# RenYurui/Global-Flow-Local-Attention

Measured on NVIDIA H100. Metric: warp-layer Mpixels/s (fwd+bwd) @256^2 C=256 k=5, higher is better.
Workload: dtype bf16

## Files before the change

global-flow-local-attention_b200/csrc/local_attn_bwd_tc.cu:

```cuda
#include <mutex>

#include "det_accum.cuh"
#include "tile_window.cuh"

namespace gfla {
namespace tc {

constexpr int BT_THREADS = 256;
constexpr int BT_PIX_REGS = 168, BT_GS_REGS = 88;
constexpr int BT_BAR_PASS = 1;
constexpr int BT_BAR_PIX = 2;
constexpr int BT_BAR_GS = 3;
constexpr int BT_BAR_FULL = 4;
constexpr int BT_BAR_FREE = 7;
constexpr int BT_AWSTR = 128 * 2 + 16;
constexpr int BT_PSTR = SEG + 1;

constexpr int BT_NAW = 3;

template <int CN>
struct BwdSmem {
    static constexpr int GSTR = CN * 2 + 16;
    static constexpr int G = 0;
    static constexpr int S = G + 128 * GSTR;
    static constexpr int AW = S + 2 * SEG * GSTR;
    static constexpr int P = AW + BT_NAW * SEG * BT_AWSTR;
    static constexpr int IRR = P + 128 * BT_PSTR * 4;
    static constexpr int ROWS = IRR + 129 * 4;
    static constexpr int ALLOC = ROWS + BT_NAW * 4;
};

__device__ __forceinline__ void red_add_16x8(__nv_bfloat16* p, const uint32_t (&v)[4]) {
    asm volatile("red.global.add.noftz.v4.bf16x2 [%0], {%1, %2, %3, %4};" ::"l"(p), "r"(v[0]), "r"(v[1]), "r"(v[2]), "r"(v[3])
                 : "memory");
}
__device__ __forceinline__ void red_add_16x8(__half* p, const uint32_t (&v)[4]) {
    asm volatile("red.global.add.noftz.v4.f16x2 [%0], {%1, %2, %3, %4};" ::"l"(p), "r"(v[0]), "r"(v[1]), "r"(v[2]), "r"(v[3])
                 : "memory");
}

__device__ __forceinline__ void quad_transpose(uint32_t (&v)[4], int t) {
    const bool t1 = (t & 2) != 0, t0 = (t & 1) != 0;
    uint32_t y0 = __shfl_xor_sync(0xffffffffu, t1 ? v[0] : v[2], 2);
    uint32_t y1 = __shfl_xor_sync(0xffffffffu, t1 ? v[1] : v[3], 2);
    if (t1) { v[0] = y0; v[1] = y1; } else { v[2] = y0; v[3] = y1; }
    y0 = __shfl_xor_sync(0xffffffffu, t0 ? v[0] : v[1], 1);
    y1 = __shfl_xor_sync(0xffffffffu, t0 ? v[2] : v[3], 1);
    if (t0) { v[0] = y0; v[2] = y1; } else { v[1] = y0; v[3] = y1; }
}

template <typename T, int CN, bool M0, bool M1>
__device__ __forceinline__ void p_gemm(uint32_t ga, uint32_t sf, float (&pacc)[2][2][4]) {
    constexpr int GSTR = BwdSmem<CN>::GSTR;
#pragma unroll 4
    for (int kk = 0; kk < CN / 16; ++kk) {
        uint32_t a0[4], a1[4], bf[4];
        if (M0) ldsm_x4(ga + kk * 32, a0);
        if (M1) ldsm_x4(ga + 16 * GSTR + kk * 32, a1);
        ldsm_x4(sf + kk * 32, bf);
        if (M0) {
            mma16<T>(pacc[0][0], a0, bf[0], bf[1]);
            mma16<T>(pacc[0][1], a0, bf[2], bf[3]);
        }
        if (M1) {
            mma16<T>(pacc[1][0], a1, bf[0], bf[1]);
            mma16<T>(pacc[1][1], a1, bf[2], bf[3]);
        }
    }
}

__device__ __forceinline__ int border_slot(int y, int x, int Hs, int Ws) {
    if (y == 0) return x;
    if (y == Hs - 1) return Ws + x;
    if (x == 0) return 2 * Ws + y;
    if (x == Ws - 1) return 2 * Ws + Hs + y;
    return -1;
}

template <typename T, int CN>
__device__ __forceinline__ void load_g_tile(uint32_t g_base, const T* __restrict__ go_b, int c0, int C, int gx0, int gy0,
                                            int H, int W, int tid) {
    constexpr int GSTR = BwdSmem<CN>::GSTR;
#pragma unroll 4
    for (int i = 0; i < CN / 16; ++i) {
        const int idx = i * BT_THREADS + tid, m = idx / (CN / 8), j = idx % (CN / 8);
        const int qx = gx0 + (m & 15), qy = gy0 + (m >> 4);
        const bool in = qx < W && qy < H;
        cp_async16(g_base + m * GSTR + j * 16, in ? go_b + ((long long)qy * W + qx) * C + c0 + j * 8 : go_b, in ? 16u : 0u);
    }
    cp_async_commit();
}

template <typename T, int K, bool DET>
__device__ __forceinline__ void irregular_pixel_bwd(const T* __restrict__ src, const float* __restrict__ flow, const T* __restrict__ logits,
                                                    const T* __restrict__ gout, T* __restrict__ gsrc, float* __restrict__ gflow,
                                                    T* __restrict__ glogits, int b, int C, int Hs, int Ws, int H, int W,
                                                    int qx, int qy, int accumulate, int lane, fx_t* __restrict__ gsum,
                                                    double2 fsc) {
    constexpr int KK = K * K;
    const long long hw = (long long)H * W, qofs = (long long)qy * W + qx;
    const float fx = flow[(long long)b * 2 * hw + qofs], fy = flow[(long long)b * 2 * hw + hw + qofs];
    float p[KK], dp[KK];
    pixel_softmax<T, float, KK>(logits + (long long)b * KK * hw + qofs, hw, KK, p);
    const float inv_kk = 1.0f / static_cast<float>(KK);
    const T* s = src + (long long)b * Hs * Ws * C;
    using GS = std::conditional_t<DET, fx_t, T>;
    GS* gs;
    if constexpr (DET) gs = gsum + (long long)b * Hs * Ws * C;
    else gs = gsrc + (long long)b * Hs * Ws * C;
    const T* go = gout + ((long long)b * hw + qofs) * C;
    float gfx = 0.f, gfy = 0.f;
#pragma unroll
    for (int i = 0; i < K; ++i) {
        const AxisTap<float> ty = axis_tap<float>(fy, i - K / 2, qy, Hs);
#pragma unroll
        for (int j = 0; j < K; ++j) {
            const AxisTap<float> tx = axis_tap<float>(fx, j - K / 2, qx, Ws);
            const long long oLT = ((long long)ty.lo * Ws + tx.lo) * C, oRT = ((long long)ty.lo * Ws + tx.hi) * C,
                            oLB = ((long long)ty.hi * Ws + tx.lo) * C, oRB = ((long long)ty.hi * Ws + tx.hi) * C;
            const float pij = p[i * K + j] * inv_kk;
            float q[4] = {0.f, 0.f, 0.f, 0.f};
            for (int c = lane; c < C; c += 32) {
                const float g = ld(go + c);
                q[0] += g * ld(s + oLT + c);
                q[1] += g * ld(s + oRT + c);
                q[2] += g * ld(s + oLB + c);
                q[3] += g * ld(s + oRB + c);
                const float gp = g * pij;
                scatter_add<DET>(gs + oLT + c, gp * (tx.wlo * ty.wlo), fsc);
                scatter_add<DET>(gs + oRT + c, gp * (tx.whi * ty.wlo), fsc);
                scatter_add<DET>(gs + oLB + c, gp * (tx.wlo * ty.whi), fsc);
                scatter_add<DET>(gs + oRB + c, gp * (tx.whi * ty.whi), fsc);
            }
#pragma unroll
            for (int t = 0; t < 4; ++t)
#pragma unroll
                for (int o = 16; o > 0; o >>= 1) q[t] += __shfl_xor_sync(0xffffffffu, q[t], o);
            dp[i * K + j] = tap_backward<float>(tx, ty, pij, inv_kk, q[0], q[1], q[2], q[3], gfx, gfy);
        }
    }
    if (lane == 0)
        store_pixel_grads<T, float, float, KK>(p, dp, KK, gfx, gfy, glogits + (long long)b * KK * hw + qofs,
                                               gflow + (long long)b * 2 * hw + qofs, hw, accumulate);
}

template <int K, int CN, bool DET, typename T>
__global__ void __launch_bounds__(BT_THREADS, 2)
k_local_attn_bwd_tc(const T* __restrict__ src, const float* __restrict__ flow, const T* __restrict__ logits, const T* __restrict__ gout,
                    T* __restrict__ gsrc, float* __restrict__ gflow, T* __restrict__ glogits, float* __restrict__ gborder, int C, int Hs, int Ws, int H, int W, int gcols,
                    int grows, int accumulate, fx_t* __restrict__ gsum, const int* __restrict__ fx_exp) {
    constexpr int K1 = K + 1, KK = K * K;
    using L = BwdSmem<CN>;
    constexpr int GSTR = L::GSTR, NTW = CN / 32;
    extern __shared__ __align__(16) unsigned char smem[];
    int* irr = reinterpret_cast<int*>(smem + L::IRR);
    int& nirr = irr[128];
    unsigned char* rows = smem + L::ROWS;
    const int tid = threadIdx.x, lane = tid & 31, warp = tid >> 5, gid = lane >> 2, tig = lane & 3;
    const float inv_kk = 1.0f / static_cast<float>(KK);
    const uint32_t sb = smem_u32(smem);
    const uint32_t g_base = sb + L::G, s_base = sb + L::S, aw_base = sb + L::AW, p_base = sb + L::P;

    for (int i = tid; i < BT_NAW * SEG * 16; i += BT_THREADS) sts128(aw_base + (i >> 4) * BT_AWSTR + (i & 15) * 16, 0u, 0u, 0u, 0u);
    if (tid == 0) nirr = 0;
    __syncthreads();
    if (warp < 4) {
        setmaxnreg_inc<BT_PIX_REGS>();
        uint32_t b;
        int gx0, gy0, bx0, by0, bx1, by1;
        group_decode(gcols, grows, b, gx0, gy0);
        group_bbox<K>(flow, b, gx0, gy0, H, W, Hs, Ws, lane, bx0, by0, bx1, by1);
        const long long hw = (long long)H * W;
        const T* go_b = gout + (long long)b * hw * C;
        const int px = gx0 + (tid & 15), py = gy0 + (tid >> 4);
        const bool valid = px < W && py < H;
        const long long pofs = (long long)py * W + px;
        uint32_t w[K1 * K1 / 2];
        float Q[K1 * K1];
#pragma unroll
        for (int i = 0; i < K1 * K1; ++i) Q[i] = 0.f;
        int X0 = 0, Y0 = 0, X0u = 0, Y0u = 0;
        bool regular = false;
        if (valid) {
            float p[KK];
            pixel_softmax<T, float, KK>(logits + (long long)b * KK * hw + pofs, hw, KK, p);
            AxisTap<float> tx[K], ty[K];
            regular = taps_regular<float, K>(flow[(long long)b * 2 * hw + pofs], flow[(long long)b * 2 * hw + hw + pofs], px, py, Hs, Ws, tx, ty);
            if (regular) {
                X0u = tx[0].fl;
                Y0u = ty[0].fl;
                build_window<T, K>(p, tx, ty, Hs, Ws, inv_kk, w, X0, Y0);
            } else {
                irr[atomicAdd(&nirr, 1)] = tid;
            }
        }
        const T* s_b = src + (long long)b * Hs * Ws * C;
        const uint32_t g_frag_a = g_base + (warp * 32 + (lane & 15)) * GSTR + (lane >> 4) * 16;
        const uint32_t s_frag_b = s_base + ((lane & 7) + ((lane >> 4) << 3)) * GSTR + ((lane >> 3) & 1) * 16;

        for (int c0 = 0; c0 < C; c0 += CN) {
            if (c0 != 0) bar_sync(BT_BAR_PASS, BT_THREADS);
            load_g_tile<T, CN>(g_base, go_b, c0, C, gx0, gy0, H, W, tid);
            {
                const int i = tid >> 3;
                for (int j = tid & 7; j < CN / 8; j += 8)
                    cp_async16(s_base + i * GSTR + j * 16, s_b + ((long long)by0 * Ws + min(bx0 + i, Ws - 1)) * C + c0 + j * 8);
            }
            cp_async_commit();
            cp_async_wait<1>();
            bar_sync(BT_BAR_PASS, BT_THREADS);
            int s = 0;
            for (int a = 0, y = by0, x = bx0; y <= by1; ++s) {
                const int buf = s & 1;
                const int an = a == BT_NAW - 1 ? 0 : a + 1;
                int xn = x + SEG, yn = y;
                if (xn > bx1) { xn = bx0; ++yn; }
                if (s >= BT_NAW) bar_sync(BT_BAR_FREE + a, BT_THREADS);
                const bool act = regular && window_meets_step<K>(X0u, Y0u, Hs, Ws, y, x);
                if (act) scatter_window_row<K>(aw_base + a * (SEG * BT_AWSTR) + tid * 2, BT_AWSTR, w, X0, Y0, y, x);
                const uint32_t pm = warp_row_bits(act);
                if (lane == 0) rows[a * 4 + warp] = static_cast<unsigned char>(pm);
                bar_arrive(BT_BAR_FULL + a, BT_THREADS);
                cp_async_wait_all();
                bar_sync(BT_BAR_PIX, 128);
                if (yn <= by1) {
                    const int i = tid >> 3;
                    const uint32_t dst = s_base + (buf ^ 1) * (SEG * GSTR) + i * GSTR;
                    const T* sp = s_b + ((long long)yn * Ws + min(xn + i, Ws - 1)) * C + c0;
                    for (int j = tid & 7; j < CN / 8; j += 8) cp_async16(dst + j * 16, sp + j * 8);
                    cp_async_commit();
                }
                if (pm != 0u) {
                    float pacc[2][2][4];
#pragma unroll
                    for (int mt = 0; mt < 2; ++mt)
#pragma unroll
                        for (int nt = 0; nt < 2; ++nt)
#pragma unroll
                            for (int q = 0; q < 4; ++q) pacc[mt][nt][q] = 0.f;
                    const uint32_t sf = s_frag_b + buf * (SEG * GSTR);
                    if (pm == 3u) p_gemm<T, CN, true, true>(g_frag_a, sf, pacc);
                    else if (pm == 1u) p_gemm<T, CN, true, false>(g_frag_a, sf, pacc);
                    else p_gemm<T, CN, false, true>(g_frag_a, sf, pacc);
#pragma unroll
                    for (int mt = 0; mt < 2; ++mt) {
                        if (((pm >> mt) & 1u) == 0u) continue;
#pragma unroll
                        for (int h = 0; h < 2; ++h) {
                            const uint32_t row = p_base + (warp * 32 + mt * 16 + gid + 8 * h) * (BT_PSTR * 4);
#pragma unroll
                            for (int nt = 0; nt < 2; ++nt) {
                                stsf(row + (nt * 8 + 2 * tig) * 4, pacc[mt][nt][2 * h]);
                                stsf(row + (nt * 8 + 2 * tig + 1) * 4, pacc[mt][nt][2 * h + 1]);
                            }
                        }
                    }
                    __syncwarp();
                    if (act) {
                        const uint32_t prow = p_base + tid * (BT_PSTR * 4);
#pragma unroll
                        for (int r = 0; r < K1; ++r) {
                            if (clampi(Y0u + r, Hs - 1) != y) continue;
#pragma unroll
                            for (int t = 0; t < K1; ++t) {
                                const int e = clampi(X0u + t, Ws - 1) - x;
                                if (e >= 0 && e < SEG) Q[r * K1 + t] += ldsf(prow + e * 4);
                            }
                        }
                    }
                }
                x = xn;
                y = yn;
                a = an;
            }
            for (int j = max(s - BT_NAW, 0); j < s; ++j) bar_sync(BT_BAR_FREE + j % BT_NAW, BT_THREADS);
        }

        if (regular) {
            float p[KK], dp[KK];
            pixel_softmax<T, float, KK>(logits + (long long)b * KK * hw + pofs, hw, KK, p);
            AxisTap<float> tx[K], ty[K];
            taps_regular<float, K>(flow[(long long)b * 2 * hw + pofs], flow[(long long)b * 2 * hw + hw + pofs], px, py, Hs, Ws, tx, ty);
            float gfx = 0.f, gfy = 0.f;
#pragma unroll
            for (int i = 0; i < K; ++i)
#pragma unroll
                for (int j = 0; j < K; ++j)
                    dp[i * K + j] = tap_backward<float>(tx[j], ty[i], p[i * K + j] * inv_kk, inv_kk, Q[i * K1 + j], Q[i * K1 + j + 1],
                                                        Q[(i + 1) * K1 + j], Q[(i + 1) * K1 + j + 1], gfx, gfy);
            store_pixel_grads<T, float, float, KK>(p, dp, KK, gfx, gfy, glogits + (long long)b * KK * hw + pofs,
                                                   gflow + (long long)b * 2 * hw + pofs, hw, accumulate);
        }
        const double2 fsc = DET ? fx_scale(fx_exp[b]) : make_double2(0.0, 0.0);
        for (int i = warp; i < nirr; i += 4) {
            const int m = irr[i];
            irregular_pixel_bwd<T, K, DET>(src, flow, logits, gout, gsrc, gflow, glogits, b, C, Hs, Ws, H, W, gx0 + (m & 15),
                                        gy0 + (m >> 4), accumulate, lane, gsum, fsc);
        }
    } else {
        setmaxnreg_dec<BT_GS_REGS>();
        uint32_t b;
        int gx0, gy0, bx0, by0, bx1, by1;
        group_decode(gcols, grows, b, gx0, gy0);
        group_bbox<K>(flow, b, gx0, gy0, H, W, Hs, Ws, lane, bx0, by0, bx1, by1);
        const long long hw = (long long)H * W;
        const T* go_b = gout + (long long)b * hw * C;
        const int v = warp - 4, t = tid - 128;
        const uint32_t aw_frag = aw_base + (lane & 15) * BT_AWSTR + (lane >> 4) * 16;
        const uint32_t g_frag_b = g_base + (lane & 15) * GSTR + (v * (CN / 4) + (lane >> 4) * 8) * 2;
        T* gs_b = gsrc + (long long)b * Hs * Ws * C;
        fx_t* gx_b = nullptr;
        double2 fsc = make_double2(0.0, 0.0);
        if constexpr (DET) {
            gx_b = gsum + (long long)b * Hs * Ws * C;
            fsc = fx_scale(fx_exp[b]);
        }

        for (int c0 = 0; c0 < C; c0 += CN) {
            if (c0 != 0) bar_sync(BT_BAR_PASS, BT_THREADS);
            load_g_tile<T, CN>(g_base, go_b, c0, C, gx0, gy0, H, W, tid);
            cp_async_wait_all();
            bar_sync(BT_BAR_PASS, BT_THREADS);
            for (int a = 0, y = by0, x = bx0; y <= by1;) {
                const int an = a == BT_NAW - 1 ? 0 : a + 1;
                int xn = x + SEG, yn = y;
                if (xn > bx1) { xn = bx0; ++yn; }
                bar_sync(BT_BAR_FULL + a, BT_THREADS);
                const uint32_t grows_on = *reinterpret_cast<const uint32_t*>(rows + a * 4);
                if (grows_on == 0u) {
                    bar_arrive(BT_BAR_FREE + a, BT_THREADS);
                } else {
                    float gacc[NTW][4];
#pragma unroll
                    for (int nt = 0; nt < NTW; ++nt)
#pragma unroll
                        for (int q = 0; q < 4; ++q) gacc[nt][q] = 0.f;
#pragma unroll
                    for (int kk = 0; kk < 128 / 16; ++kk) {
                        if (((grows_on >> (8 * (kk >> 1) + (kk & 1))) & 1u) == 0u) continue;
                        uint32_t af[4];
                        ldsm_x4(aw_frag + a * (SEG * BT_AWSTR) + kk * 32, af);
#pragma unroll
                        for (int np = 0; np < NTW / 2; ++np) {
                            uint32_t bg[4];
                            ldsm_x4_t(g_frag_b + kk * 16 * GSTR + np * 32, bg);
                            mma16<T>(gacc[2 * np], af, bg[0], bg[1]);
                            mma16<T>(gacc[2 * np + 1], af, bg[2], bg[3]);
                        }
                    }
                    bar_sync(BT_BAR_GS, 128);
                    {
                        const uint32_t z = aw_base + a * (SEG * BT_AWSTR) + (t >> 3) * BT_AWSTR + (t & 7) * 32;
                        sts128(z, 0u, 0u, 0u, 0u);
                        sts128(z + 16, 0u, 0u, 0u, 0u);
                    }
                    bar_arrive(BT_BAR_FREE + a, BT_THREADS);
                    if constexpr (DET) {
#pragma unroll
                        for (int h = 0; h < 2; ++h) {
                            const int xp = x + gid + 8 * h;
                            fx_t* d = gx_b + ((long long)y * Ws + xp) * C + c0 + v * (CN / 4);
                            const bool t0 = (tig & 1) != 0;
#pragma unroll
                            for (int j = 0; j < NTW / 2; ++j) {
                                const float a0 = gacc[2 * j][2 * h], a1 = gacc[2 * j][2 * h + 1];
                                const float b0 = gacc[2 * j + 1][2 * h], b1 = gacc[2 * j + 1][2 * h + 1];
                                const float r0 = __shfl_xor_sync(0xffffffffu, t0 ? a0 : b0, 1);
                                const float r1 = __shfl_xor_sync(0xffffffffu, t0 ? a1 : b1, 1);
                                uint32_t u[4];
                                u[0] = __float_as_uint(t0 ? r0 : a0);
                                u[1] = __float_as_uint(t0 ? r1 : a1);
                                u[2] = __float_as_uint(t0 ? b0 : r0);
                                u[3] = __float_as_uint(t0 ? b1 : r1);
                                quad_transpose(u, tig);
                                if (xp <= bx1) {
#pragma unroll
                                    for (int n = 0; n < 4; ++n)
                                        fx_add(d + (2 * j + (n & 1)) * 8 + 4 * (n >> 1) + tig, __uint_as_float(u[n]), fsc);
                                }
                            }
                        }
                    } else {
                        uint32_t gv[2 * NTW];
#pragma unroll
                        for (int h = 0; h < 2; ++h) {
                            const int xp = x + gid + 8 * h;
                            const int slot = xp > bx1 ? -2 : border_slot(y, xp, Hs, Ws);
                            if (slot >= 0) {
                                float* d = gborder + ((long long)b * 2 * (Hs + Ws) + slot) * C + c0 + v * (CN / 4) + 2 * tig;
#pragma unroll
                                for (int nt = 0; nt < NTW; ++nt) {
                                    const float v0 = gacc[nt][2 * h], v1 = gacc[nt][2 * h + 1];
                                    if (v0 != 0.f || v1 != 0.f) atomicAdd(reinterpret_cast<float2*>(d + nt * 8), make_float2(v0, v1));
                                }
                            }
#pragma unroll
                            for (int nt = 0; nt < NTW; ++nt) {
                                const typename Pair16<T>::type hv = floats2_rn<T>(gacc[nt][2 * h], gacc[nt][2 * h + 1]);
                                gv[h * NTW + nt] = slot == -1 ? *reinterpret_cast<const uint32_t*>(&hv) : 0u;
                            }
                        }
#pragma unroll
                        for (int j = 0; j < NTW / 2; ++j) {
                            uint32_t u[4] = {gv[4 * j], gv[4 * j + 1], gv[4 * j + 2], gv[4 * j + 3]};
                            quad_transpose(u, tig);
                            if ((u[0] | u[1] | u[2] | u[3]) != 0u) {
                                const int n = 4 * j + tig, h = n / NTW, nt = n % NTW;
                                red_add_16x8(gs_b + ((long long)y * Ws + x + gid + 8 * h) * C + c0 + v * (CN / 4) + nt * 8, u);
                            }
                        }
                    }
                }
                x = xn;
                y = yn;
                a = an;
            }
        }
    }
}

template <typename T>
__global__ void __launch_bounds__(256)
k_fold_border(T* __restrict__ gsrc, const float* __restrict__ gborder, int B, int C, int Hs, int Ws) {
    const int nb = 2 * (Hs + Ws), c2 = C / 2;
    const long long i = (long long)blockIdx.x * blockDim.x + threadIdx.x;
    if (i >= (long long)B * nb * c2) return;
    const long long bs = i / c2;
    const int c = (int)(i % c2) * 2, s = (int)(bs % nb), b = (int)(bs / nb);
    int y, x;
    if (s < Ws) { y = 0; x = s; }
    else if (s < 2 * Ws) { y = Hs - 1; x = s - Ws; }
    else if (s < 2 * Ws + Hs) { y = s - 2 * Ws; x = 0; }
    else { y = s - 2 * Ws - Hs; x = Ws - 1; }
    if (border_slot(y, x, Hs, Ws) != s) return;
    const float2 v = *reinterpret_cast<const float2*>(gborder + bs * C + c);
    typename Pair16<T>::type* d = reinterpret_cast<typename Pair16<T>::type*>(gsrc + (((long long)b * Hs + y) * Ws + x) * C + c);
    const float2 o = pair_to_float2(*d);
    *d = floats2_rn<T>(o.x + v.x, o.y + v.y);
}

template <int K, int CN, bool DET, typename T>
static int launch_bwd(const void* src, const void* flow, const void* logits, const void* gout, void* gsrc, void* gflow, void* glogits,
                      float* gborder, int B, int C, int Hs, int Ws, int H, int W, int accumulate, cudaStream_t st_,
                      fx_t* gsum = nullptr, const int* fx_exp = nullptr) {
    const int gcols = (W + GW - 1) / GW, grows = (H + GH - 1) / GH;
    const long long ngroups = (long long)B * gcols * grows;
    if (ngroups > INT_MAX) return GFLA_E_SHAPE;
    auto kern = k_local_attn_bwd_tc<K, CN, DET, T>;
    cudaError_t e = cudaFuncSetAttribute(kern, cudaFuncAttributeMaxDynamicSharedMemorySize, BwdSmem<CN>::ALLOC);
    if (e != cudaSuccess) return static_cast<int>(e);
    kern<<<(unsigned)ngroups, BT_THREADS, BwdSmem<CN>::ALLOC, st_>>>(
        (const T*)src, (const float*)flow, (const T*)logits, (const T*)gout, (T*)gsrc, (float*)gflow, (T*)glogits, gborder, C, Hs, Ws, H, W, gcols, grows, accumulate, gsum, fx_exp);
    const int st = launch_status();
    if (st != GFLA_OK || DET) return st;
    const long long n = (long long)B * 2 * (Hs + Ws) * (C / 2);
    k_fold_border<T><<<(unsigned)((n + 255) / 256), 256, 0, st_>>>((T*)gsrc, gborder, B, C, Hs, Ws);
    return launch_status();
}

}

static cudaError_t scratch_alloc(void** p, size_t bytes, cudaStream_t st_) {
    static std::mutex mu;
    static cudaMemPool_t pools[64] = {};
    int dev = 0;
    cudaError_t e = cudaGetDevice(&dev);
    if (e != cudaSuccess) return e;
    if (dev >= 64) return cudaMallocAsync(p, bytes, st_);
    {
        std::lock_guard<std::mutex> lock(mu);
        if (pools[dev] == nullptr) {
            cudaMemPoolProps props = {};
            props.allocType = cudaMemAllocationTypePinned;
            props.location.type = cudaMemLocationTypeDevice;
            props.location.id = dev;
            e = cudaMemPoolCreate(&pools[dev], &props);
            if (e != cudaSuccess) { pools[dev] = nullptr; return e; }
            uint64_t keep = UINT64_MAX;
            e = cudaMemPoolSetAttribute(pools[dev], cudaMemPoolAttrReleaseThreshold, &keep);
            if (e != cudaSuccess) return e;
        }
    }
    return cudaMallocFromPoolAsync(p, bytes, pools[dev], st_);
}

static int pick_cn_bwd(int C) {
    if (C % 256 == 0) return 256;
    if (C == 128 || C == 64) return C;
    return 0;
}

bool local_attn_bwd_tc_supported(int C, int k, int dtype, int flow_dtype, int layout, const void* src, const void* gout,
                                 const void* gsrc) {
    return (dtype == GFLA_BF16 || dtype == GFLA_F16) && flow_dtype == GFLA_F32 && layout == GFLA_NHWC && (k == 3 || k == 5) && pick_cn_bwd(C) != 0 &&
           aligned(src, 16) && aligned(gout, 16) && aligned(gsrc, 16);
}

int local_attn_bwd_tc(const void* src, const void* flow, const void* logits, const void* gout, void* gsrc, void* gflow, void* glogits,
                      int B, int C, int Hs, int Ws, int H, int W, int k, int dtype, int accumulate, cudaStream_t st_) {
    if (!accumulate) {
        const int z = zero_async(gsrc, (size_t)B * C * Hs * Ws * 2, st_);
        if (z != GFLA_OK) return z;
    }
    const int cn = pick_cn_bwd(C);
    if (cn == 0 || (k != 3 && k != 5)) return GFLA_E_NOTSUP;
    const size_t border_bytes = (size_t)B * 2 * (Hs + Ws) * C * sizeof(float);
    float* gborder = nullptr;
    cudaError_t e = scratch_alloc(reinterpret_cast<void**>(&gborder), border_bytes, st_);
    if (e != cudaSuccess) return static_cast<int>(e);
    int r = zero_async(gborder, border_bytes, st_);
    if (r == GFLA_OK) {
#define GFLA_BT_CASE(T_, K_, CN_) \
        if (k == K_ && cn == CN_) r = tc::launch_bwd<K_, CN_, false, T_>(src, flow, logits, gout, gsrc, gflow, glogits, gborder, B, C, Hs, Ws, H, W, accumulate, st_);
        if (dtype == GFLA_F16) {
            GFLA_BT_CASE(__half, 5, 256) GFLA_BT_CASE(__half, 5, 128) GFLA_BT_CASE(__half, 5, 64)
            GFLA_BT_CASE(__half, 3, 256) GFLA_BT_CASE(__half, 3, 128) GFLA_BT_CASE(__half, 3, 64)
        } else {
            GFLA_BT_CASE(__nv_bfloat16, 5, 256) GFLA_BT_CASE(__nv_bfloat16, 5, 128) GFLA_BT_CASE(__nv_bfloat16, 5, 64)
            GFLA_BT_CASE(__nv_bfloat16, 3, 256) GFLA_BT_CASE(__nv_bfloat16, 3, 128) GFLA_BT_CASE(__nv_bfloat16, 3, 64)
        }
#undef GFLA_BT_CASE
    }
    e = cudaFreeAsync(gborder, st_);
    return r != GFLA_OK ? r : static_cast<int>(e);
}

int local_attn_bwd_tc_det(const void* src, const void* flow, const void* logits, const void* gout, void* gflow, void* glogits, int B,
                          int C, int Hs, int Ws, int H, int W, int k, int dtype, int accumulate, fx_t* gsum, const int* fx_exp,
                          cudaStream_t st_) {
    const int cn = pick_cn_bwd(C);
#define GFLA_BT_CASE(T_, K_, CN_) \
    if (k == K_ && cn == CN_) return tc::launch_bwd<K_, CN_, true, T_>(src, flow, logits, gout, nullptr, gflow, glogits, nullptr, B, C, Hs, \
                                                                       Ws, H, W, accumulate, st_, gsum, fx_exp);
    if (dtype == GFLA_F16) {
        GFLA_BT_CASE(__half, 5, 256) GFLA_BT_CASE(__half, 5, 128) GFLA_BT_CASE(__half, 5, 64)
        GFLA_BT_CASE(__half, 3, 256) GFLA_BT_CASE(__half, 3, 128) GFLA_BT_CASE(__half, 3, 64)
    } else {
        GFLA_BT_CASE(__nv_bfloat16, 5, 256) GFLA_BT_CASE(__nv_bfloat16, 5, 128) GFLA_BT_CASE(__nv_bfloat16, 5, 64)
        GFLA_BT_CASE(__nv_bfloat16, 3, 256) GFLA_BT_CASE(__nv_bfloat16, 3, 128) GFLA_BT_CASE(__nv_bfloat16, 3, 64)
    }
#undef GFLA_BT_CASE
    return GFLA_E_NOTSUP;
}

}
```

global-flow-local-attention_b200/csrc/tc_common.cuh:

```cuda
#pragma once
#include <cuda_bf16.h>
#include <cuda_fp16.h>
#include <cuda_runtime.h>
#include <stdint.h>

#include "gfla_warp.h"

namespace gfla {
namespace tc {

__device__ __forceinline__ uint32_t smem_u32(const void* p) { return static_cast<uint32_t>(__cvta_generic_to_shared(p)); }

__device__ __forceinline__ void sts128(uint32_t a, uint32_t x, uint32_t y, uint32_t z, uint32_t w) {
    asm volatile("st.shared.v4.b32 [%0], {%1, %2, %3, %4};" ::"r"(a), "r"(x), "r"(y), "r"(z), "r"(w) : "memory");
}
__device__ __forceinline__ void sts16(uint32_t a, uint32_t v) {
    asm volatile("{\n\t.reg .b16 h;\n\tcvt.u16.u32 h, %1;\n\tst.shared.b16 [%0], h;\n\t}" ::"r"(a), "r"(v) : "memory");
}
__device__ __forceinline__ void stsf(uint32_t a, float v) { asm volatile("st.shared.f32 [%0], %1;" ::"r"(a), "f"(v) : "memory"); }
__device__ __forceinline__ float ldsf(uint32_t a) {
    float v;
    asm volatile("ld.shared.f32 %0, [%1];" : "=f"(v) : "r"(a) : "memory");
    return v;
}

__device__ __forceinline__ void cp_async16(uint32_t dst, const void* src, uint32_t src_bytes = 16) {
    asm volatile("cp.async.cg.shared.global [%0], [%1], 16, %2;" ::"r"(dst), "l"(src), "r"(src_bytes) : "memory");
}
__device__ __forceinline__ void cp_async_commit() { asm volatile("cp.async.commit_group;" ::: "memory"); }
__device__ __forceinline__ void cp_async_wait_all() { asm volatile("cp.async.wait_group 0;" ::: "memory"); }
template <int N>
__device__ __forceinline__ void cp_async_wait() { asm volatile("cp.async.wait_group %0;" ::"n"(N) : "memory"); }

__device__ __forceinline__ void ldsm_x4(uint32_t a, uint32_t (&r)[4]) {
    asm volatile("ldmatrix.sync.aligned.m8n8.x4.shared.b16 {%0, %1, %2, %3}, [%4];"
                 : "=r"(r[0]), "=r"(r[1]), "=r"(r[2]), "=r"(r[3]) : "r"(a) : "memory");
}
__device__ __forceinline__ void ldsm_x4_t(uint32_t a, uint32_t (&r)[4]) {
    asm volatile("ldmatrix.sync.aligned.m8n8.x4.trans.shared.b16 {%0, %1, %2, %3}, [%4];"
                 : "=r"(r[0]), "=r"(r[1]), "=r"(r[2]), "=r"(r[3]) : "r"(a) : "memory");
}
__device__ __forceinline__ void mma_bf16(float (&d)[4], const uint32_t (&a)[4], uint32_t b0, uint32_t b1) {
    asm volatile(
        "mma.sync.aligned.m16n8k16.row.col.f32.bf16.bf16.f32 {%0, %1, %2, %3}, {%4, %5, %6, %7}, {%8, %9}, {%0, %1, %2, %3};"
        : "+f"(d[0]), "+f"(d[1]), "+f"(d[2]), "+f"(d[3])
        : "r"(a[0]), "r"(a[1]), "r"(a[2]), "r"(a[3]), "r"(b0), "r"(b1));
}

__device__ __forceinline__ void bar_sync(int id, int n) { asm volatile("bar.sync %0, %1;" ::"r"(id), "r"(n) : "memory"); }
__device__ __forceinline__ void bar_arrive(int id, int n) { asm volatile("bar.arrive %0, %1;" ::"r"(id), "r"(n) : "memory"); }
template <int N>
__device__ __forceinline__ void setmaxnreg_inc() { asm volatile("setmaxnreg.inc.sync.aligned.u32 %0;" ::"n"(N)); }
template <int N>
__device__ __forceinline__ void setmaxnreg_dec() { asm volatile("setmaxnreg.dec.sync.aligned.u32 %0;" ::"n"(N)); }

__device__ __forceinline__ uint32_t bf16_bits(float v) {
    const __nv_bfloat16 h = __float2bfloat16_rn(v);
    return static_cast<uint32_t>(*reinterpret_cast<const unsigned short*>(&h));
}

__device__ __forceinline__ void mma_f16(float (&d)[4], const uint32_t (&a)[4], uint32_t b0, uint32_t b1) {
    asm volatile(
        "mma.sync.aligned.m16n8k16.row.col.f32.f16.f16.f32 {%0, %1, %2, %3}, {%4, %5, %6, %7}, {%8, %9}, {%0, %1, %2, %3};"
        : "+f"(d[0]), "+f"(d[1]), "+f"(d[2]), "+f"(d[3])
        : "r"(a[0]), "r"(a[1]), "r"(a[2]), "r"(a[3]), "r"(b0), "r"(b1));
}
__device__ __forceinline__ uint32_t f16_bits(float v) {
    const __half h = __float2half_rn(v);
    return static_cast<uint32_t>(*reinterpret_cast<const unsigned short*>(&h));
}

template <typename T> struct Pair16;
template <> struct Pair16<__nv_bfloat16> { using type = __nv_bfloat162; };
template <> struct Pair16<__half> { using type = __half2; };

template <typename T> __device__ __forceinline__ void mma16(float (&d)[4], const uint32_t (&a)[4], uint32_t b0, uint32_t b1);
template <> __device__ __forceinline__ void mma16<__nv_bfloat16>(float (&d)[4], const uint32_t (&a)[4], uint32_t b0, uint32_t b1) {
    mma_bf16(d, a, b0, b1);
}
template <> __device__ __forceinline__ void mma16<__half>(float (&d)[4], const uint32_t (&a)[4], uint32_t b0, uint32_t b1) {
    mma_f16(d, a, b0, b1);
}
template <typename T> __device__ __forceinline__ uint32_t bits16(float v);
template <> __device__ __forceinline__ uint32_t bits16<__nv_bfloat16>(float v) { return bf16_bits(v); }
template <> __device__ __forceinline__ uint32_t bits16<__half>(float v) { return f16_bits(v); }
template <typename T> __device__ __forceinline__ typename Pair16<T>::type floats2_rn(float a, float b);
template <> __device__ __forceinline__ __nv_bfloat162 floats2_rn<__nv_bfloat16>(float a, float b) { return __floats2bfloat162_rn(a, b); }
template <> __device__ __forceinline__ __half2 floats2_rn<__half>(float a, float b) { return __floats2half2_rn(a, b); }
__device__ __forceinline__ float2 pair_to_float2(__nv_bfloat162 v) { return __bfloat1622float2(v); }
__device__ __forceinline__ float2 pair_to_float2(__half2 v) { return __half22float2(v); }

struct FastDiv {
    uint32_t d, mul, shr;
    __device__ __forceinline__ void init(uint32_t div) {
        d = div;
        if (div <= 1) { mul = 0; shr = 0; return; }
        const uint32_t p = 31 + (32 - __clz(div - 1));
        mul = static_cast<uint32_t>(((1ull << p) + div - 1) / div);
        shr = p - 32;
    }
    __device__ __forceinline__ uint32_t div(uint32_t n) const { return d != 1 ? __umulhi(n, mul) >> shr : n; }
    __device__ __forceinline__ void divmod(uint32_t n, uint32_t& q, uint32_t& r) const { q = div(n); r = n - q * d; }
};

}
}
```

global-flow-local-attention_b200/csrc/tile_window.cuh:

```cuda
#pragma once
#include <climits>

#include "local_attn_pixel.cuh"
#include "tc_common.cuh"

namespace gfla {
namespace tc {

constexpr int GW = 16, GH = 8;
constexpr int SEG = 16;

__device__ __forceinline__ void group_decode(int gcols, int grows, uint32_t& b, int& gx0, int& gy0) {
    FastDiv fc, fr;
    fc.init(gcols);
    fr.init(grows);
    uint32_t g = blockIdx.x, gc, gr;
    fc.divmod(g, g, gc);
    fr.divmod(g, b, gr);
    gx0 = gc * GW;
    gy0 = gr * GH;
}

template <int K>
__device__ __forceinline__ void group_bbox(const float* __restrict__ flow, int b, int gx0, int gy0, int H, int W, int Hs,
                                           int Ws, int lane, int& x0, int& y0, int& x1, int& y1) {
    const long long hw = (long long)H * W;
    float rfx[4], rfy[4];
#pragma unroll
    for (int i = 0; i < 4; ++i) {
        const int m = lane + 32 * i, px = gx0 + (m & 15), py = gy0 + (m >> 4);
        const bool valid = px < W && py < H;
        const long long o = (long long)b * 2 * hw + (long long)py * W + px;
        rfx[i] = valid ? flow[o] : 0.f;
        rfy[i] = valid ? flow[o + hw] : 0.f;
    }
    int xmin = INT_MAX, xmax = INT_MIN, ymin = INT_MAX, ymax = INT_MIN;
#pragma unroll
    for (int i = 0; i < 4; ++i) {
        const int m = lane + 32 * i, px = gx0 + (m & 15), py = gy0 + (m >> 4);
        if (px < W && py < H) {
            xmin = min(xmin, axis_tap<float>(rfx[i], -(K / 2), px, Ws).lo);
            xmax = max(xmax, axis_tap<float>(rfx[i], K - 1 - K / 2, px, Ws).hi);
            ymin = min(ymin, axis_tap<float>(rfy[i], -(K / 2), py, Hs).lo);
            ymax = max(ymax, axis_tap<float>(rfy[i], K - 1 - K / 2, py, Hs).hi);
        }
    }
#pragma unroll
    for (int o = 16; o > 0; o >>= 1) {
        xmin = min(xmin, __shfl_xor_sync(0xffffffffu, xmin, o));
        xmax = max(xmax, __shfl_xor_sync(0xffffffffu, xmax, o));
        ymin = min(ymin, __shfl_xor_sync(0xffffffffu, ymin, o));
        ymax = max(ymax, __shfl_xor_sync(0xffffffffu, ymax, o));
    }
    x0 = xmin; y0 = ymin; x1 = xmax; y1 = ymax;
}

template <typename T, int K>
__device__ __forceinline__ void build_window(const float* p, const AxisTap<float> (&tx)[K], const AxisTap<float> (&ty)[K],
                                             int Hs, int Ws, float scale, uint32_t (&wp)[(K + 1) * (K + 1) / 2], int& X0, int& Y0) {
    constexpr int K1 = K + 1;
    float w[K1 * K1];
#pragma unroll
    for (int i = 0; i < K1 * K1; ++i) w[i] = 0.f;
#pragma unroll
    for (int i = 0; i < K; ++i) {
        float rowx[K1];
#pragma unroll
        for (int s = 0; s < K1; ++s) rowx[s] = 0.f;
#pragma unroll
        for (int j = 0; j < K; ++j) {
            const float pij = p[i * K + j] * scale;
            rowx[j] += pij * tx[j].wlo;
            rowx[j + 1] += pij * tx[j].whi;
        }
#pragma unroll
        for (int s = 0; s < K1; ++s) {
            w[i * K1 + s] += ty[i].wlo * rowx[s];
            w[(i + 1) * K1 + s] += ty[i].whi * rowx[s];
        }
    }
    X0 = tx[0].fl;
    Y0 = ty[0].fl;
    if (X0 < 0 || X0 + K > Ws - 1 || Y0 < 0 || Y0 + K > Hs - 1) {
#pragma unroll
        for (int r = 0; r < K1; ++r) {
#pragma unroll
            for (int s = 0; s < K; ++s)
                if (X0 + s < 0) { w[r * K1 + s + 1] += w[r * K1 + s]; w[r * K1 + s] = 0.f; }
#pragma unroll
            for (int s = K; s > 0; --s)
                if (X0 + s > Ws - 1) { w[r * K1 + s - 1] += w[r * K1 + s]; w[r * K1 + s] = 0.f; }
        }
#pragma unroll
        for (int s = 0; s < K1; ++s) {
#pragma unroll
            for (int r = 0; r < K; ++r)
                if (Y0 + r < 0) { w[(r + 1) * K1 + s] += w[r * K1 + s]; w[r * K1 + s] = 0.f; }
#pragma unroll
            for (int r = K; r > 0; --r)
                if (Y0 + r > Hs - 1) { w[(r - 1) * K1 + s] += w[r * K1 + s]; w[r * K1 + s] = 0.f; }
        }
        X0 = min(max(X0, -K), Ws - 1);
        Y0 = min(max(Y0, -K), Hs - 1);
    }
#pragma unroll
    for (int i = 0; i < K1 * K1 / 2; ++i) wp[i] = bits16<T>(w[2 * i]) | (bits16<T>(w[2 * i + 1]) << 16);
}

template <int K, int NPOS = SEG>
__device__ __forceinline__ void scatter_window_row(uint32_t base, uint32_t stride, const uint32_t (&wp)[(K + 1) * (K + 1) / 2],
                                                   int X0, int Y0, int y, int x) {
    constexpr int K1 = K + 1, RW = K1 / 2;
    const int rr = y - Y0;
    if (rr < 0 || rr > K) return;
    uint32_t wr[RW];
#pragma unroll
    for (int s = 0; s < RW; ++s) wr[s] = 0u;
#pragma unroll
    for (int r = 0; r < K1; ++r)
        if (rr == r) {
#pragma unroll
            for (int s = 0; s < RW; ++s) wr[s] = wp[r * RW + s];
        }
#pragma unroll
    for (int s = 0; s < K1; ++s) {
        const int e = X0 + s - x;
        const uint32_t h = (s & 1) ? wr[s / 2] >> 16 : wr[s / 2] & 0xffffu;
        if (e >= 0 && e < NPOS && (h & 0x7fffu) != 0u) sts16(base + e * stride, h);
    }
}

template <int K>
__device__ __forceinline__ bool window_meets_step(int X0, int Y0, int Hs, int Ws, int y, int x) {
    return clampi(Y0, Hs - 1) <= y && y <= clampi(Y0 + K, Hs - 1) && clampi(X0, Ws - 1) < x + SEG && clampi(X0 + K, Ws - 1) >= x;
}

__device__ __forceinline__ uint32_t warp_row_bits(bool active) {
    const uint32_t bal = __ballot_sync(0xffffffffu, active);
    return ((bal & 0xffffu) != 0u ? 1u : 0u) | ((bal >> 16) != 0u ? 2u : 0u);
}

template <typename T, int K, bool NHWC>
__device__ __forceinline__ void irregular_pixel(const T* __restrict__ src, const T* __restrict__ logits, T* __restrict__ out,
                                                const T* __restrict__ prev, const T* __restrict__ mask, int b, int C, int Hs, int Ws,
                                                int H, int W,
                                                int qx, int qy, float qfx, float qfy, int lane) {
    constexpr int KK = K * K;
    const long long hw = (long long)H * W, qofs = (long long)qy * W + qx;
    float p[KK];
    pixel_softmax<T, float, KK>(logits + (long long)b * KK * hw + qofs, hw, KK, p);
    const long long spl = (long long)Hs * Ws;
    const long long sc = NHWC ? 1 : spl, sp = NHWC ? C : 1;
    const T* sb = src + (long long)b * spl * C;
    T* ob = NHWC ? out + ((long long)b * hw + qofs) * C : out + (long long)b * C * hw + qofs;
    for (int c = lane; c < C; c += 32) {
        const T* s = sb + c * sc;
        float acc = 0.f;
#pragma unroll 1
        for (int i = 0; i < K; ++i) {
            const AxisTap<float> ty = axis_tap<float>(qfy, i - K / 2, qy, Hs);
#pragma unroll 1
            for (int j = 0; j < K; ++j) {
                const AxisTap<float> tx = axis_tap<float>(qfx, j - K / 2, qx, Ws);
                acc += p[i * K + j] * tap_value(s, tx, ty, Ws, sp);
            }
        }
        acc *= 1.0f / static_cast<float>(KK);
        if (prev != nullptr) {
            const float qm = ld(mask + (long long)b * hw + qofs);
            const T* pb = NHWC ? prev + ((long long)b * hw + qofs) * C : prev + (long long)b * C * hw + qofs;
            acc = ld(pb + (NHWC ? (long long)c : (long long)c * hw)) * (1.f - qm) + acc * qm;
        }
        st(ob + (NHWC ? (long long)c : (long long)c * hw), acc);
    }
}

}
}
```

Before: 277.1.

## Triple-buffer source segments in backward kernel and skip empty half-tile MMAs

Source segment loads in the tensor-core backward kernel move from a double buffer to a three-slot ring. Two segments are prefetched before the loop, and the wait relaxes from wait_all to wait<1>, so the load for the segment two steps ahead overlaps with the current GEMM. It also adds an N1 template flag: when the trailing 8-column half of a segment lies past the row end, it uses ldmatrix x2 and skips the second-N MMAs and P stores. The cost is extra shared memory for the third segment buffer, which may lower occupancy, and more template instantiations.

```diff
diff --git a/global-flow-local-attention_b200/csrc/local_attn_bwd_tc.cu b/global-flow-local-attention_b200/csrc/local_attn_bwd_tc.cu
--- a/global-flow-local-attention_b200/csrc/local_attn_bwd_tc.cu
+++ b/global-flow-local-attention_b200/csrc/local_attn_bwd_tc.cu
@@ -17,13 +17,14 @@
 constexpr int BT_PSTR = SEG + 1;
 
 constexpr int BT_NAW = 3;
+constexpr int BT_NSEG = 3;
 
 template <int CN>
 struct BwdSmem {
     static constexpr int GSTR = CN * 2 + 16;
     static constexpr int G = 0;
     static constexpr int S = G + 128 * GSTR;
-    static constexpr int AW = S + 2 * SEG * GSTR;
+    static constexpr int AW = S + BT_NSEG * SEG * GSTR;
     static constexpr int P = AW + BT_NAW * SEG * BT_AWSTR;
     static constexpr int IRR = P + 128 * BT_PSTR * 4;
     static constexpr int ROWS = IRR + 129 * 4;
@@ -49,7 +50,7 @@
     if (t0) { v[0] = y0; v[2] = y1; } else { v[1] = y0; v[3] = y1; }
 }
 
-template <typename T, int CN, bool M0, bool M1>
+template <typename T, int CN, bool M0, bool M1, bool N1>
 __device__ __forceinline__ void p_gemm(uint32_t ga, uint32_t sf, float (&pacc)[2][2][4]) {
     constexpr int GSTR = BwdSmem<CN>::GSTR;
 #pragma unroll 4
@@ -57,14 +58,15 @@
         uint32_t a0[4], a1[4], bf[4];
         if (M0) ldsm_x4(ga + kk * 32, a0);
         if (M1) ldsm_x4(ga + 16 * GSTR + kk * 32, a1);
-        ldsm_x4(sf + kk * 32, bf);
+        if (N1) ldsm_x4(sf + kk * 32, bf);
+        else ldsm_x2(sf + kk * 32, bf[0], bf[1]);
         if (M0) {
             mma16<T>(pacc[0][0], a0, bf[0], bf[1]);
-            mma16<T>(pacc[0][1], a0, bf[2], bf[3]);
+            if (N1) mma16<T>(pacc[0][1], a0, bf[2], bf[3]);
         }
         if (M1) {
             mma16<T>(pacc[1][0], a1, bf[0], bf[1]);
-            mma16<T>(pacc[1][1], a1, bf[2], bf[3]);
+            if (N1) mma16<T>(pacc[1][1], a1, bf[2], bf[3]);
         }
     }
 }
@@ -89,6 +91,14 @@
         cp_async16(g_base + m * GSTR + j * 16, in ? go_b + ((long long)qy * W + qx) * C + c0 + j * 8 : go_b, in ? 16u : 0u);
     }
     cp_async_commit();
+}
+
+template <typename T, int CN>
+__device__ __forceinline__ void load_segment(uint32_t dst, const T* __restrict__ s_b, int c0, int C, int Ws, int y, int x, int tid) {
+    constexpr int GSTR = BwdSmem<CN>::GSTR;
+    const int i = tid >> 3;
+    const T* sp = s_b + ((long long)y * Ws + min(x + i, Ws - 1)) * C + c0;
+    for (int j = tid & 7; j < CN / 8; j += 8) cp_async16(dst + i * GSTR + j * 16, sp + j * 8);
 }
 
 template <typename T, int K, bool DET>
@@ -201,18 +211,22 @@
         for (int c0 = 0; c0 < C; c0 += CN) {
             if (c0 != 0) bar_sync(BT_BAR_PASS, BT_THREADS);
             load_g_tile<T, CN>(g_base, go_b, c0, C, gx0, gy0, H, W, tid);
-            {
-                const int i = tid >> 3;
-                for (int j = tid & 7; j < CN / 8; j += 8)
-                    cp_async16(s_base + i * GSTR + j * 16, s_b + ((long long)by0 * Ws + min(bx0 + i, Ws - 1)) * C + c0 + j * 8);
+            int fy = by0, fx = bx0;
+#pragma unroll
+            for (int i = 0; i < 2; ++i) {
+                if (fy <= by1) {
+                    load_segment<T, CN>(s_base + i * (SEG * GSTR), s_b, c0, C, Ws, fy, fx, tid);
+                    fx += SEG;
+                    if (fx > bx1) { fx = bx0; ++fy; }
+                }
+                cp_async_commit();
             }
-            cp_async_commit();
-            cp_async_wait<1>();
+            cp_async_wait<2>();
             bar_sync(BT_BAR_PASS, BT_THREADS);
             int s = 0;
-            for (int a = 0, y = by0, x = bx0; y <= by1; ++s) {
-                const int buf = s & 1;
+            for (int a = 0, sl = 0, y = by0, x = bx0; y <= by1; ++s) {
                 const int an = a == BT_NAW - 1 ? 0 : a + 1;
+                const int sn = sl == BT_NSEG - 1 ? 0 : sl + 1;
                 int xn = x + SEG, yn = y;
                 if (xn > bx1) { xn = bx0; ++yn; }
                 if (s >= BT_NAW) bar_sync(BT_BAR_FREE + a, BT_THREADS);
@@ -221,15 +235,14 @@
                 const uint32_t pm = warp_row_bits(act);
                 if (lane == 0) rows[a * 4 + warp] = static_cast<unsigned char>(pm);
                 bar_arrive(BT_BAR_FULL + a, BT_THREADS);
-                cp_async_wait_all();
+                cp_async_wait<1>();
                 bar_sync(BT_BAR_PIX, 128);
-                if (yn <= by1) {
-                    const int i = tid >> 3;
-                    const uint32_t dst = s_base + (buf ^ 1) * (SEG * GSTR) + i * GSTR;
-                    const T* sp = s_b + ((long long)yn * Ws + min(xn + i, Ws - 1)) * C + c0;
-                    for (int j = tid & 7; j < CN / 8; j += 8) cp_async16(dst + j * 16, sp + j * 8);
-                    cp_async_commit();
+                if (fy <= by1) {
+                    load_segment<T, CN>(s_base + (sn == BT_NSEG - 1 ? 0 : sn + 1) * (SEG * GSTR), s_b, c0, C, Ws, fy, fx, tid);
+                    fx += SEG;
+                    if (fx > bx1) { fx = bx0; ++fy; }
                 }
+                cp_async_commit();
                 if (pm != 0u) {
                     float pacc[2][2][4];
 #pragma unroll
@@ -238,10 +251,17 @@
                         for (int nt = 0; nt < 2; ++nt)
 #pragma unroll
                             for (int q = 0; q < 4; ++q) pacc[mt][nt][q] = 0.f;
-                    const uint32_t sf = s_frag_b + buf * (SEG * GSTR);
-                    if (pm == 3u) p_gemm<T, CN, true, true>(g_frag_a, sf, pacc);
-                    else if (pm == 1u) p_gemm<T, CN, true, false>(g_frag_a, sf, pacc);
-                    else p_gemm<T, CN, false, true>(g_frag_a, sf, pacc);
+                    const uint32_t sf = s_frag_b + sl * (SEG * GSTR);
+                    const bool n1 = x + 8 <= bx1;
+                    if (n1) {
+                        if (pm == 3u) p_gemm<T, CN, true, true, true>(g_frag_a, sf, pacc);
+                        else if (pm == 1u) p_gemm<T, CN, true, false, true>(g_frag_a, sf, pacc);
+                        else p_gemm<T, CN, false, true, true>(g_frag_a, sf, pacc);
+                    } else {
+                        if (pm == 3u) p_gemm<T, CN, true, true, false>(g_frag_a, sf, pacc);
+                        else if (pm == 1u) p_gemm<T, CN, true, false, false>(g_frag_a, sf, pacc);
+                        else p_gemm<T, CN, false, true, false>(g_frag_a, sf, pacc);
+                    }
 #pragma unroll
                     for (int mt = 0; mt < 2; ++mt) {
                         if (((pm >> mt) & 1u) == 0u) continue;
@@ -250,6 +270,7 @@
                             const uint32_t row = p_base + (warp * 32 + mt * 16 + gid + 8 * h) * (BT_PSTR * 4);
 #pragma unroll
                             for (int nt = 0; nt < 2; ++nt) {
+                                if (nt == 1 && !n1) continue;
                                 stsf(row + (nt * 8 + 2 * tig) * 4, pacc[mt][nt][2 * h]);
                                 stsf(row + (nt * 8 + 2 * tig + 1) * 4, pacc[mt][nt][2 * h + 1]);
                             }
@@ -272,6 +293,7 @@
                 x = xn;
                 y = yn;
                 a = an;
+                sl = sn;
             }
             for (int j = max(s - BT_NAW, 0); j < s; ++j) bar_sync(BT_BAR_FREE + j % BT_NAW, BT_THREADS);
         }
diff --git a/global-flow-local-attention_b200/csrc/tc_common.cuh b/global-flow-local-attention_b200/csrc/tc_common.cuh
--- a/global-flow-local-attention_b200/csrc/tc_common.cuh
+++ b/global-flow-local-attention_b200/csrc/tc_common.cuh
@@ -39,6 +39,9 @@
 __device__ __forceinline__ void ldsm_x4_t(uint32_t a, uint32_t (&r)[4]) {
     asm volatile("ldmatrix.sync.aligned.m8n8.x4.trans.shared.b16 {%0, %1, %2, %3}, [%4];"
                  : "=r"(r[0]), "=r"(r[1]), "=r"(r[2]), "=r"(r[3]) : "r"(a) : "memory");
+}
+__device__ __forceinline__ void ldsm_x2(uint32_t a, uint32_t& r0, uint32_t& r1) {
+    asm volatile("ldmatrix.sync.aligned.m8n8.x2.shared.b16 {%0, %1}, [%2];" : "=r"(r0), "=r"(r1) : "r"(a) : "memory");
 }
 __device__ __forceinline__ void mma_bf16(float (&d)[4], const uint32_t (&a)[4], uint32_t b0, uint32_t b1) {
     asm volatile(
```

New measurement: 279.6, median of 6. About the same (+0.9%).

## Move AW buffer clearing to pixel warps and double-buffer gather ldmatrix loads

Applied to the files above, without the earlier changes.

The gsrc warps no longer zero the whole attention-weight buffer after their MMAs, which needed an extra 128-thread named barrier. Instead each pixel thread, after the free barrier, clears only the sparse entries it previously scattered into that buffer. The gsrc MMA loop also double-buffers the transposed ldmatrix loads of the gradient tile so the next fragment load overlaps the current MMAs. This shortens the consumer warps' critical path at the cost of extra per-thread clearing work and bookkeeping on the producer side.

```diff
diff --git a/global-flow-local-attention_b200/csrc/local_attn_bwd_tc.cu b/global-flow-local-attention_b200/csrc/local_attn_bwd_tc.cu
--- a/global-flow-local-attention_b200/csrc/local_attn_bwd_tc.cu
+++ b/global-flow-local-attention_b200/csrc/local_attn_bwd_tc.cu
@@ -10,7 +10,6 @@
 constexpr int BT_PIX_REGS = 168, BT_GS_REGS = 88;
 constexpr int BT_BAR_PASS = 1;
 constexpr int BT_BAR_PIX = 2;
-constexpr int BT_BAR_GS = 3;
 constexpr int BT_BAR_FULL = 4;
 constexpr int BT_BAR_FREE = 7;
 constexpr int BT_AWSTR = 128 * 2 + 16;
@@ -210,12 +209,21 @@
             cp_async_wait<1>();
             bar_sync(BT_BAR_PASS, BT_THREADS);
             int s = 0;
+            int yc = by0, xc = bx0;
+            auto clear_step = [&](int a) {
+                if (regular) clear_window_row<K>(aw_base + a * (SEG * BT_AWSTR) + tid * 2, BT_AWSTR, X0, Y0, yc, xc);
+                xc += SEG;
+                if (xc > bx1) { xc = bx0; ++yc; }
+            };
             for (int a = 0, y = by0, x = bx0; y <= by1; ++s) {
                 const int buf = s & 1;
                 const int an = a == BT_NAW - 1 ? 0 : a + 1;
                 int xn = x + SEG, yn = y;
                 if (xn > bx1) { xn = bx0; ++yn; }
-                if (s >= BT_NAW) bar_sync(BT_BAR_FREE + a, BT_THREADS);
+                if (s >= BT_NAW) {
+                    bar_sync(BT_BAR_FREE + a, BT_THREADS);
+                    clear_step(a);
+                }
                 const bool act = regular && window_meets_step<K>(X0u, Y0u, Hs, Ws, y, x);
                 if (act) scatter_window_row<K>(aw_base + a * (SEG * BT_AWSTR) + tid * 2, BT_AWSTR, w, X0, Y0, y, x);
                 const uint32_t pm = warp_row_bits(act);
@@ -273,7 +281,10 @@
                 y = yn;
                 a = an;
             }
-            for (int j = max(s - BT_NAW, 0); j < s; ++j) bar_sync(BT_BAR_FREE + j % BT_NAW, BT_THREADS);
+            for (int j = max(s - BT_NAW, 0); j < s; ++j) {
+                bar_sync(BT_BAR_FREE + j % BT_NAW, BT_THREADS);
+                clear_step(j % BT_NAW);
+            }
         }
 
         if (regular) {
@@ -305,7 +316,7 @@
         group_bbox<K>(flow, b, gx0, gy0, H, W, Hs, Ws, lane, bx0, by0, bx1, by1);
         const long long hw = (long long)H * W;
         const T* go_b = gout + (long long)b * hw * C;
-        const int v = warp - 4, t = tid - 128;
+        const int v = warp - 4;
         const uint32_t aw_frag = aw_base + (lane & 15) * BT_AWSTR + (lane >> 4) * 16;
         const uint32_t g_frag_b = g_base + (lane & 15) * GSTR + (v * (CN / 4) + (lane >> 4) * 8) * 2;
         T* gs_b = gsrc + (long long)b * Hs * Ws * C;
@@ -340,19 +351,15 @@
                         if (((grows_on >> (8 * (kk >> 1) + (kk & 1))) & 1u) == 0u) continue;
                         uint32_t af[4];
                         ldsm_x4(aw_frag + a * (SEG * BT_AWSTR) + kk * 32, af);
+                        const uint32_t g_k = g_frag_b + kk * 16 * GSTR;
+                        uint32_t bg[2][4];
+                        ldsm_x4_t(g_k, bg[0]);
 #pragma unroll
                         for (int np = 0; np < NTW / 2; ++np) {
-                            uint32_t bg[4];
-                            ldsm_x4_t(g_frag_b + kk * 16 * GSTR + np * 32, bg);
-                            mma16<T>(gacc[2 * np], af, bg[0], bg[1]);
-                            mma16<T>(gacc[2 * np + 1], af, bg[2], bg[3]);
+                            if (np + 1 < NTW / 2) ldsm_x4_t(g_k + (np + 1) * 32, bg[(np + 1) & 1]);
+                            mma16<T>(gacc[2 * np], af, bg[np & 1][0], bg[np & 1][1]);
+                            mma16<T>(gacc[2 * np + 1], af, bg[np & 1][2], bg[np & 1][3]);
                         }
-                    }
-                    bar_sync(BT_BAR_GS, 128);
-                    {
-                        const uint32_t z = aw_base + a * (SEG * BT_AWSTR) + (t >> 3) * BT_AWSTR + (t & 7) * 32;
-                        sts128(z, 0u, 0u, 0u, 0u);
-                        sts128(z + 16, 0u, 0u, 0u, 0u);
                     }
                     bar_arrive(BT_BAR_FREE + a, BT_THREADS);
                     if constexpr (DET) {
diff --git a/global-flow-local-attention_b200/csrc/tile_window.cuh b/global-flow-local-attention_b200/csrc/tile_window.cuh
--- a/global-flow-local-attention_b200/csrc/tile_window.cuh
+++ b/global-flow-local-attention_b200/csrc/tile_window.cuh
@@ -130,6 +130,17 @@
     }
 }
 
+template <int K, int NPOS = SEG>
+__device__ __forceinline__ void clear_window_row(uint32_t base, uint32_t stride, int X0, int Y0, int y, int x) {
+    const int rr = y - Y0;
+    if (rr < 0 || rr > K) return;
+#pragma unroll
+    for (int s = 0; s < K + 1; ++s) {
+        const int e = X0 + s - x;
+        if (e >= 0 && e < NPOS) sts16(base + e * stride, 0u);
+    }
+}
+
 template <int K>
 __device__ __forceinline__ bool window_meets_step(int X0, int Y0, int Hs, int Ws, int y, int x) {
     return clampi(Y0, Hs - 1) <= y && y <= clampi(Y0 + K, Hs - 1) && clampi(X0, Ws - 1) < x + SEG && clampi(X0 + K, Ws - 1) >= x;
```

Result: no change. 277.1 before, 277.5 after (median of 6 runs) (+0.2%).
